# TzuYaoHuang/WaterLily.jl

Hardware: AMD Instinct MI355X
Metric: cells*steps/sec (3D TGV) ; smoother HBM GB/s vs peak (higher is better)
Workload: dtype f32; 1 GPU; 3D Taylor-Green vortex 512^3 Float32, wall-bounded, Re=1600, NoBody, remeasure=false (BASELINE configs[4] domain on 1 GPU); size=512, resjac=630, resjac_redo=0

## Files before the change

include/wlhip_bench.h:

```cpp
#ifndef WLHIP_BENCH_H
#define WLHIP_BENCH_H
#include "wlhip.h"
#ifdef __cplusplus
extern "C" {
#endif

enum { WL_PROF_GS_SWEEP = 0, WL_PROF_SMOOTH = 1, WL_PROF_JACOBI = 2, WL_PROF_CONVDIFF = 3, WL_PROF_RESIDUAL = 4,
       WL_PROF_BDIM = 5, WL_PROF_PROLONG = 6, WL_PROF_COARSE = 7, WL_PROF_STEP = 8, WL_PROF_GS_A = 9, WL_PROF_GS_B = 10, WL_PROF_NSLOTS = 11 };
int wl_prof_enable(int on);
int wl_prof_read(int slot, int* host_count, double* host_total_ms);

long wl_launch_count(void);
int wl_placement_scores(double* out, int cap);
int wl_sim_counter(wl_sim* s, const char* name, long* out);

#ifdef __cplusplus
}
#endif
#endif
```

waterlily.jl_amd/_lib.py:

```python
import ctypes as C
import os

_HERE = os.path.dirname(os.path.abspath(__file__))
LIB_PATH = os.environ.get("WLHIP_LIB") or os.path.join(_HERE, "libwlhip.so")


class wl_grid(C.Structure):
    _fields_ = [("D", C.c_int32), ("nx", C.c_int32), ("ny", C.c_int32), ("nz", C.c_int32),
                ("k0", C.c_int32), ("k1", C.c_int32), ("gk", C.c_int32), ("gnz", C.c_int32)]


class wl_body(C.Structure):
    _fields_ = [("kind", C.c_int32), ("c", C.c_float * 3), ("R", C.c_float), ("m", C.c_float * 3), ("V", C.c_float * 3)]


def make_body(body, D):
    name = body[0]
    pad = lambda v: [float(x) for x in v] + [0.0] * (3 - len(v))
    b = wl_body()
    if name == "sphere":
        b.kind, b.R, m, rest = 1, float(body[2]), [1.0] * D, body[3:]
    elif name == "cylinder":
        b.kind, b.R, m, rest = 1, float(body[2]), [0.0 if k == int(body[3]) else 1.0 for k in range(D)], body[4:]
    elif name == "plane":
# ... 138 lines not shown
    "wl_comm_set_periodic": (i32, [P, i32]),
    "wl_comm_halo_async": (i32, [P, P, G, i32, i32, P]),
    "wl_comm_combine_test": (i32, [P, P, P, P]),
    "wl_comm_destroy": (i32, [P]),
    "wl_comm_rank": (i32, [P]),
    "wl_comm_size": (i32, [P]),
    "wl_comm_stats": (i32, [P, C.POINTER(C.c_int64)]),
    "wl_halo_exchange": (i32, [P, P, G, i32, i32, P]),
    "wl_allgather_planes": (i32, [P, P, G, i32, P]),
    "wl_grid_slab": (i32, [G, i32, C.POINTER(C.c_int32), i32, i32, i32]),
    "wl_sim_create_slab": (i32, [C.POINTER(P), C.POINTER(wl_sim_desc), P]),
    "wl_launch_count": (C.c_long, []),
    "wl_reset_process_options": (i32, []),
    "wl_placement_scores": (i32, [C.POINTER(C.c_double), i32]),
    "wl_sim_counter": (i32, [P, C.c_char_p, C.POINTER(C.c_long)]),
    "wl_prof_enable": (i32, [i32]),
    "wl_prof_read": (i32, [i32, C.POINTER(i32), C.POINTER(f64)]),
    "wl_sim_pressure_force_sphere": (i32, [P, C.POINTER(f32), f32, C.POINTER(f64), P]),
    "wl_measure_body": (i32, [P, P, P, P, G, C.POINTER(wl_body), f32, i32, C.c_uint32, P]),
    "wl_pressure_force_body": (i32, [P, G, C.POINTER(wl_body), C.POINTER(f64), P]),
    "wl_viscous_force_body": (i32, [P, G, f32, C.POINTER(wl_body), C.POINTER(f64), P]),
    "wl_pressure_moment_body": (i32, [C.POINTER(f32), P, G, C.POINTER(wl_body), C.POINTER(f64), P]),
    "wl_viscous_moment_body": (i32, [C.POINTER(f32), P, G, f32, C.POINTER(wl_body), C.POINTER(f64), P]),
    "wl_sim_pressure_moment_body": (i32, [P, C.POINTER(f32), C.POINTER(wl_body), C.POINTER(f64), P]),
    "wl_sim_viscous_moment_body": (i32, [P, C.POINTER(f32), C.POINTER(wl_body), C.POINTER(f64), P]),
    "wl_sim_measure_body": (i32, [P, C.POINTER(wl_body), f32, P]),
    "wl_sim_pressure_force_body": (i32, [P, C.POINTER(wl_body), C.POINTER(f64), P]),
    "wl_sim_viscous_force_body": (i32, [P, C.POINTER(wl_body), C.POINTER(f64), P]),
    "wl_bodyset_measure_points": (i32, [C.POINTER(wl_bodyset), i32, C.POINTER(f32), i32, f32, C.POINTER(f32), C.POINTER(f32), C.POINTER(f32), P]),
    "wl_measure_bodyset": (i32, [P, P, P, P, G, C.POINTER(wl_bodyset), f32, i32, C.c_uint32, P]),
# ... 49 lines not shown
```

waterlily.jl_amd/csrc/wl_mg.hip:

```cpp
#include <cmath>
#include <cstdlib>
#include <utility>

#include "wl_common.hpp"
#include "wl_mg.hpp"

bool wl_mg_divisible(int n) { return (n % 2 == 0) && n > 4; }

int wl_mg::build(float* x, float* L, float* z, const wl_grid& g0, unsigned per, int maxlevels, wl_comm* c) {
  perdir = per; comm = (c && c->size > 1) ? c : nullptr;
  WL_TRY(wl_ctx_ensure());
  WL_HIP(hipMalloc(&red, wl_red_bytes()));
  ws = wl_red_ws(red);
  const bool dist0 = comm && g0.D == 3 && g0.nz != g0.gnz;
  if (dist0 && ((per >> 2) & 1u) && !comm->zperiodic) { wl_set_error("z-periodic z-slabs need a communicator in periodic mode (wl_comm_set_periodic)"); return WL_EINVAL; }
  std::vector<wl_grid> grids; std::vector<char> isdist; std::vector<wl_grid> views; std::vector<char> hasview;
  grids.push_back(g0); isdist.push_back(dist0); views.push_back(g0); hasview.push_back(0);
  while ((int)grids.size() <= maxlevels) {
    const wl_grid f = grids.back(); const bool fd = isdist.back();
    const bool cx = wl_mg_divisible(f.nx), cy = wl_mg_divisible(f.ny), cz = (f.D == 3) && wl_mg_divisible(f.gnz);
    if (!(cx || cy || cz)) break;
    wl_grid cgr = f; wl_grid vw = f; bool cd = fd, hv = false;
    if (cx) cgr.nx = 1 + f.nx / 2;
    if (cy) cgr.ny = 1 + f.ny / 2;
// ... 271 lines not shown
  }
  WL_TRY(halo(fine, fine.r, 1, s));
  if (l == 0 && shift_pending) { shift_pending = false; WL_TRY(wl::jacobi_pp_shift(fine.eps, fine.r, fine.x, fine.x_, 1.f, fine.cl, ws, WL_RD_L1_INIT, WL_RF_LINF_INIT, s)); }
  else {
    const int xz = fine.xzero ? 1 : 0; fine.xzero = false;
    if (zsplit_ranges(fine).on) {
      ZPart parts[3]; zsplit_parts(*this, fine, parts);
      for (int i = 0; i < 3; i++) if (parts[i].any()) WL_TRY(wl::jacobi_pp(fine.eps, fine.r, fine.x, fine.L, fine.D, fine.iD, parts[i].of(fine.x_), 1.f, *parts[i].cl, s, xz));
    } else WL_TRY(wl::jacobi_pp(fine.eps, fine.r, fine.x, fine.L, fine.D, fine.iD, fine.x_, 1.f, fine.cl, s, xz));
  }
  std::swap(fine.r, fine.eps);
  return 0;
}
int wl_mg::restrict_to_coarse(int l, bool to_tail, hipStream_t s) {
  Level& fine = lv[(size_t)l]; Level& coarse = lv[(size_t)l + 1];
  if (coarse.has_view) {
    WL_TRY(wl::restrict_(coarse.r, coarse.view, fine.r, fine.x_, s));
    WL_TRY(wl::allgather_planes(comm, coarse.r, coarse.view, 1, s));
  } else WL_TRY(wl::restrict_(coarse.r, coarse.x_, fine.r, fine.x_, s));
  coarse.xzero = skip_fill && !to_tail && l + 2 < (int)lv.size() && !perdir && !coarse.dist && !coarse.has_view;
  return coarse.xzero ? 0 : wl::fill(coarse.x, 0.f, (size_t)coarse.x_.cs, s);
}
int wl_mg::descend(int l, bool to_tail, float w, hipStream_t s) {
  Level& fine = lv[(size_t)l]; Level& coarse = lv[(size_t)l + 1];
  if (to_tail) WL_TRY(tail(l + 1, w, s));
  else {
    if (l + 2 < (int)lv.size()) WL_TRY(vcycle(l + 1, w, s, true));
    WL_TRY(smooth(l + 1, 4, w, s, false, nullptr, skip_r ? wl::B_XONLY : wl::B_BOTH));
  }
  return halo(coarse, coarse.x, 1, s, coarse_x_depth(fine, coarse));
}
// ... 96 lines not shown
```

waterlily.jl_amd/csrc/wl_mg.hpp:

```cpp
#pragma once
#include <algorithm>
#include <functional>
#include <vector>

#include "wl_comm.hpp"

bool wl_mg_divisible(int n);
struct WlNormSlots { int d, f; };
inline constexpr WlNormSlots WL_ZS_NORMS[3] = {{WL_RD_L1, WL_RF_LINF}, {WL_RD_L1_Z1, WL_RF_LINF_Z1}, {WL_RD_L1_Z2, WL_RF_LINF_Z2}};

struct wl_mg {
  struct Level {
    wl_grid g; GridX x_;
    float *L = nullptr, *D = nullptr, *iD = nullptr, *x = nullptr, *eps = nullptr, *r = nullptr, *z = nullptr;
    float *em = nullptr, *rs = nullptr;
    float* wx = nullptr;
    wl::ConstL cl{};
    bool xzero = false;
    bool part = false; int za = 0, zb = -1; wl::ConstL clp{};
    bool pend = false;
    bool dist = false;
    GridX view;
    bool has_view = false;
  };
// ... 18 lines not shown
  bool use_zsplit = true;
  long zsplit_min = 16L << 20;
  bool skip_fill = true;
  bool defer_shift = true;
  bool shift_pending = false;
  bool deep_halo = true;
  struct Spec {
    std::function<int(const float*)> tail; int check_head = 0; bool tail_stood = false, head_decided = false, head_due = false;
    void disarm() { tail = nullptr; check_head = 0; }
    void begin_solve(std::function<int(const float*)>* t, int* check) { t->swap(tail); *check = check_head; disarm(); tail_stood = head_decided = head_due = false; }
  } spec;
  int shift_path = -1;
  hipStream_t side = nullptr; hipEvent_t ev_decided = nullptr;
  double first_hd0 = 0.0;
  bool jacobi0_done = false;
  int norm_slots = 0;
  bool par_ranges = false;
  int x_halo_depth = 1;
  int last_xdefer = -1;
  bool use_xdefer = true;
  bool use_wide = true;
  bool overlap_smooth = true;
  bool use_tail = true;
  bool tail_ok(int first) const;
  int tail(int first, float w, hipStream_t s);
  float* slab = nullptr;
  void* red = nullptr;
  RedWs ws;
  std::vector<double> log_r1, log_rinf, log_w;

// ... 46 lines not shown
```

waterlily.jl_amd/csrc/wl_pdefer.hpp:

```cpp
#pragma once
#include "wl_common.hpp"

#ifdef __HIPCC__
__device__ __forceinline__ float wl_unscale(float x, float dt) { return x / dt; }
#endif

namespace wl {
int resjac(float* xout, float* rout, const float* x, const float* u, const GridX& g, float dt, float w, const ConstL& cl, const RedWs& ws, int slot_d, int slot_f, hipStream_t s,
           bool shell, const float* bcU, float dt_prev);
int project_unscale(float* u, const float* L, const float* x, float* pout, const GridX& g, float dt, const ConstL& cl, hipStream_t s, const BcFold* fold, bool skip_p);
int project_cfl(float* uout, const float* uin, const float* L, const float* x, float* pout, float* sigma, const GridX& g, float dt, const ConstL& cl, const RedWs& ws, int slot_f, hipStream_t s,
                int store_sigma, const BcFold* fold, bool skip_p);
}
```

waterlily.jl_amd/csrc/wl_resjac.hip:

```cpp
#include <cstdlib>

#include "wl_common.hpp"
#include "wl_pdefer.hpp"

namespace {

__device__ __forceinline__ float rj_cf(int Ia, int Na, float c) { return (Ia <= 2 || Ia >= Na) ? 0.f : c; }
__device__ __forceinline__ float rj_inv(float d) { return (d == 0.f) ? d : 1.0f / d; }
__device__ __forceinline__ float2 rj_ld2(const float* __restrict__ p, unsigned o) { return *reinterpret_cast<const float2*>(p + o); }
__device__ __forceinline__ void rj_st2(float* __restrict__ p, unsigned o, float2 v, bool s0, bool s1) {
  if (s0 && s1) *reinterpret_cast<float2*>(p + o) = v;
  else { if (s0) p[o] = v.x; if (s1) p[o + 1] = v.y; }
}
struct RjBc { int on; float U[3]; };
int g_resjac_on = 1;
long g_resjac_min = 6L << 20;

#define RJ_Y 32
#define RJ_NS rj32
#include "wl_resjac_body.inc"
#undef RJ_Y
#undef RJ_NS
#define RJ_Y 16
#define RJ_NS rj16
// ... 58 lines not shown
  return g_resjac_on && cl.on && g.D == 3 && (g.nz == g.gnz ? g.gk == 0 : (g.k0 >= 2 && g.nz - g.k1 >= 2 && g.k1 - g.k0 >= 8)) && (g.nx & 1) == 0 && g.nx >= 66 && g.ny >= 34 &&
         g.gnz >= 10 && g.cs < (1L << 30) && (long)(g.nx - 2) * (g.ny - 2) * (g.gnz - 2) >= g_resjac_min;
}
int shell_nonzero(const float* a, const GridX& g, int* dev_flag, hipStream_t s) {
  WL_HIP(hipMemsetAsync(dev_flag, 0, sizeof(int), s));
  hipLaunchKernelGGL(k_shell_nonzero, dim3(8, (unsigned)g.nz), dim3(WL_BLOCK), 0, s, g, a, dev_flag);
  int h = 1;
  WL_HIP(hipMemcpyAsync(&h, dev_flag, sizeof(int), hipMemcpyDeviceToHost, s));
  WL_HIP(hipStreamSynchronize(s));
  return h ? 1 : 0;
}
int resjac(float* xout, float* rout, const float* x, const float* u, const GridX& g, float dt, float w, const ConstL& cl, const RedWs& ws, int slot_d, int slot_f, hipStream_t s, bool shell, const float* bcU) {
  return resjac(xout, rout, x, u, g, dt, w, cl, ws, slot_d, slot_f, s, shell, bcU, 0.f);
}
int resjac(float* xout, float* rout, const float* x, const float* u, const GridX& g, float dt, float w, const ConstL& cl, const RedWs& ws, int slot_d, int slot_f, hipStream_t s, bool shell, const float* bcU, float dt_prev) {
  if (xout == x) { wl_set_error("resjac: output aliases input"); return WL_EINVAL; }
  const int np = g.k1 - g.k0;
  static const int rows_env = wl_exp_int("WL_RJ_ROWS", 0);
  const bool r16 = rows_env != 32;
  const int ntiles = r16 ? rj16::rj_tiles(g) : rj32::rj_tiles(g), per = (ntiles + 7) >> 3;
  const long SX = r16 ? rj16::rj_slots_per_xcd() : rj32::rj_slots_per_xcd();
  static const int envc = wl_exp_int("WL_RJ_CHUNK", 0);
  int zc = envc;
  if (zc <= 0) {
    static const int chforce = wl_exp_int("WL_RJ_CHUNKS", 0);
    double best = -1.0; zc = np;
    for (int chunks = 1; chunks <= np; chunks++) {
      const int z = (np + chunks - 1) / chunks;
      if (z < 8) break;
      const long W = (long)per * ((np + z - 1) / z), rounds = (W + SX - 1) / SX;
      double cost = (double)rounds * (z + 2) * (1.0 + 0.3 / (double)rounds);
      if (W < SX) cost = (z + 2) * 1.3;
      if (chforce > 0) cost = (chunks == chforce) ? 0.0 : 1e30;
      if (best < 0 || cost < best) { best = cost; zc = z; }
    }
  }
  if (zc > np) zc = np;
  const int nch = (np + zc - 1) / zc;
  const unsigned nb = (unsigned)(8 * per * nch);
  if (nb > WL_MAXPART) { wl_set_error("resjac: too many workgroups for the reduction workspace"); return WL_EINVAL; }
  if (dt_prev != 0.f && !(dt_prev > 0.f && dt > 0.f)) { wl_set_error("resjac: a pending unscale needs positive Δt"); return WL_EINVAL; }
  if (shell) hipLaunchKernelGGL(k_scale_shell, dim3(8, (unsigned)g.nz), dim3(WL_BLOCK), 0, s, g, xout, x, dt, dt_prev);
  RjBc bc{0, {0.f, 0.f, 0.f}};
  if (bcU) { if (g.nz != g.gnz) { wl_set_error("resjac: BC! on load is for the single domain"); return WL_EINVAL; } bc.on = 1; for (int a = 0; a < 3; a++) bc.U[a] = bcU[a]; }
  if (r16) rj16::rj_launch(nb, s, g, xout, rout, x, u, dt, dt_prev, w, cl, zc, ws.pa, ws.pb, ws.pm, bc);
  else rj32::rj_launch(nb, s, g, xout, rout, x, u, dt, dt_prev, w, cl, zc, ws.pa, ws.pb, ws.pm, bc);
  hipLaunchKernelGGL(k_resjac_fin, dim3(1), dim3(WL_BLOCK), 0, s, (const double*)ws.pa, (const double*)ws.pb, (const float*)ws.pm, (int)nb, ws.res_d, ws.res_f, slot_d, slot_f);
  WL_LAUNCH_CHECK(); return 0;
}
}
```

waterlily.jl_amd/csrc/wl_resjac_body.inc:

```
#define RJ_X 32
#define RJ_N (RJ_X * RJ_Y)
#define RJ_W (RJ_X + 2)
#define RJ_H ((RJ_Y + 2) * RJ_W)
#define RJ_SZ (2 * RJ_H)
#define RJ_HX 2
#define RJ_HY 2
#define RJ_CX (2 * RJ_X - 2 * RJ_HX)
#define RJ_CY (RJ_Y - 2 * RJ_HY)
namespace RJ_NS {
#ifndef RJ_WAVES
#define RJ_WAVES 8
#endif
template <int PEND>
__global__ void __launch_bounds__(RJ_N, RJ_WAVES) k_resjac(GridX g, float* __restrict__ xout, float* __restrict__ rout, const float* __restrict__ p, const float* __restrict__ u,
                                                    float dt, float dt_prev, float w, wl::ConstL cl, int zchunk, double* __restrict__ psum, double* __restrict__ pl1, float* __restrict__ pmax, RjBc bc) {
  __shared__ float sX[2][RJ_SZ];
  __shared__ float sE[2][RJ_SZ];
  const int ntx = (g.nx - 1 + RJ_CX - 1) / RJ_CX, nty = (g.ny - 2 + RJ_CY - 1) / RJ_CY;
  const int ntiles = ntx * nty;
  const unsigned h = blockIdx.x, q = h & 7u, sblk = h >> 3;
  const unsigned per = (unsigned)((ntiles + 7) >> 3);
  const int c = (int)(sblk / per);
  const int tl = (int)(q * per + (sblk - (unsigned)c * per));
  double nsum = 0.0, nl1 = 0.0; float nmax = 0.f;
  const int ks = g.k0 + c * zchunk, ke = (ks + zchunk < g.k1) ? ks + zchunk : g.k1;
  if (tl < ntiles && ks < ke) {
    const int tx = tl % ntx, ty = tl / ntx;
    const int lx = threadIdx.x % RJ_X, ly = threadIdx.x / RJ_X;
    const int i0 = tx * RJ_CX - RJ_HX + 2 * lx, j = 1 + ty * RJ_CY - RJ_HY + ly;
    const int lq = (ly + 1) * RJ_W + lx + 1;
    const bool indom = i0 >= 0 && i0 <= g.nx - 2 && j >= 0 && j < g.ny;
    const bool jin = j >= 1 && j <= g.ny - 2;
    const bool in0 = indom && jin && i0 >= 2, in1 = indom && jin && i0 + 1 <= g.nx - 2;
    const bool corep = 2 * lx >= RJ_HX && 2 * lx < 2 * RJ_X - RJ_HX && ly >= RJ_HY && ly < RJ_Y - RJ_HY;
    const bool st0 = corep && in0, st1 = corep && in1;
    const unsigned oc = indom ? (unsigned)i0 + (unsigned)j * (unsigned)g.sy : 0u;
    const unsigned sz = (unsigned)g.sz, cs = (unsigned)g.cs;
    for (int qq = threadIdx.x; qq < RJ_SZ; qq += RJ_N) { sX[0][qq] = 0.f; sX[1][qq] = 0.f; sE[0][qq] = 0.f; sE[1][qq] = 0.f; }
    const float cxa = rj_cf(i0 + 1, g.nx, cl.c[0]), cxb = rj_cf(i0 + 2, g.nx, cl.c[0]), cxc = rj_cf(i0 + 3, g.nx, cl.c[0]);
    const float ky = rj_cf(j + 1, g.ny, cl.c[1]), kyp = rj_cf(j + 2, g.ny, cl.c[1]);
    float dxy0 = 0.f; dxy0 -= (cxa + cxb); dxy0 -= (ky + kyp);
    float dxy1 = 0.f; dxy1 -= (cxb + cxc); dxy1 -= (ky + kyp);
    const float c2 = cl.c[2];
    const int oth0 = RJ_H + lq - 1, oth1 = lq + 1;
    auto plane_ok = [&](int K) { return K >= 0 && K <= g.nz - 1; };
    auto ldp = [&](int K) -> float2 {
      if (!(indom && plane_ok(K))) return make_float2(0.f, 0.f);
      const float2 v = rj_ld2(p, oc + (unsigned)K * sz);
      if (PEND) return make_float2(wl_unscale(v.x, dt_prev) * dt, wl_unscale(v.y, dt_prev) * dt);
      return make_float2(v.x * dt, v.y * dt);
    };
    const bool sbx = bc.on && (i0 == 0 || i0 == g.nx - 2);
    const bool sby = bc.on && j == 1, sbyp = bc.on && j + 1 == g.ny - 1;
    auto lduz = [&](int K) -> float2 {
      if (!(indom && plane_ok(K) && (in0 || in1))) return make_float2(0.f, 0.f);
      if (bc.on && (g.gk + K == 1 || g.gk + K == g.gnz - 1)) return make_float2(bc.U[2], bc.U[2]);
      return rj_ld2(u, 2u * cs + oc + (unsigned)K * sz);
    };
    const int K0 = ks - 1;
    float2 xm = ldp(K0 - 1), x0 = ldp(K0), xp;
    float2 uz0 = lduz(K0), uzp;
    float2 em1 = {0.f, 0.f}, e0 = em1, e1 = em1;
    float2 r1 = em1, r0 = em1;
    __syncthreads();
    sX[K0 & 1][lq] = x0.x; sX[K0 & 1][lq + RJ_H] = x0.y;
    for (int K = K0; K <= ke; K++) {
      xp = ldp(K + 1); uzp = lduz(K + 1);
      const bool planeK = g.gk + K >= 1 && g.gk + K <= g.gnz - 2 && K >= 1 && K <= g.nz - 2;
      float2 ux = {0.f, 0.f}, uy = ux, uyp = ux; float uxr = 0.f;
      if (planeK && (in0 || in1)) {
        const unsigned o = oc + (unsigned)K * sz;
        ux = rj_ld2(u, o); uxr = u[o + 2];
        uy = rj_ld2(u, cs + o); uyp = rj_ld2(u, cs + o + (unsigned)g.sy);
// ... 24 lines not shown
          e1.x = r0.x * id0;
        }
        if (in1) {
          float dv = 0.f;
          dv += uxr - ux.y;
          dv += uyp.y - uy.y;
          dv += uzp.y - uz0.y;
          float s = x0.y * d1;
          s += (x0.x * cxb + SX[oth1] * cxc);
          s += (SX[RJ_H + lq - RJ_W] * ky + SX[RJ_H + lq + RJ_W] * kyp);
          s += (xm.y * lz + xp.y * lzp);
          r0.y = (d1 == 0.f) ? 0.f : dv - s;
          e1.y = r0.y * id1;
        }
        if (K >= ks && K < ke) {
          const float a0 = st0 ? r0.x : 0.f, a1 = st1 ? r0.y : 0.f;
          nsum += (double)a0; nsum += (double)a1;
          nl1 += (double)fabsf(a0); nl1 += (double)fabsf(a1); nmax = fmaxf(nmax, fmaxf(fabsf(a0), fabsf(a1)));
        }
      }
      sE[K & 1][lq] = e1.x; sE[K & 1][lq + RJ_H] = e1.y;
      const int P = K - 1;
      if (P >= ks && P < ke && (st0 || st1)) {
        const float* __restrict__ SE = sE[P & 1];
        const float lzP = rj_cf(g.gk + P + 1, g.gnz, c2), lzpP = lz;
        const float zsP = lzP + lzpP;
        float2 rn, xn;
        {
          float s = e0.x * (dxy0 - zsP);
          s += (SE[oth0] * cxa + e0.y * cxb);
          s += (SE[lq - RJ_W] * ky + SE[lq + RJ_W] * kyp);
          s += (em1.x * lzP + e1.x * lzpP);
          rn.x = r1.x - w * s; xn.x = xm.x + w * e0.x;
        }
        {
          float s = e0.y * (dxy1 - zsP);
          s += (e0.x * cxb + SE[oth1] * cxc);
          s += (SE[RJ_H + lq - RJ_W] * ky + SE[RJ_H + lq + RJ_W] * kyp);
          s += (em1.y * lzP + e1.y * lzpP);
          rn.y = r1.y - w * s; xn.y = xm.y + w * e0.y;
        }
        const unsigned oP = oc + (unsigned)P * sz;
        rj_st2(rout, oP, rn, st0, st1);
        rj_st2(xout, oP, xn, st0, st1);
      }
      xm = x0; x0 = xp; uz0 = uzp;
    }
  }
  __shared__ double shs[RJ_N / 64], shl[RJ_N / 64]; __shared__ float shm[RJ_N / 64];
  nsum = wave_sum(nsum); nl1 = wave_sum(nl1); nmax = wave_max(nmax);
  __syncthreads();
  if ((threadIdx.x & 63) == 0) { shs[threadIdx.x >> 6] = nsum; shl[threadIdx.x >> 6] = nl1; shm[threadIdx.x >> 6] = nmax; }
  __syncthreads();
  if (threadIdx.x == 0) {
    double a = 0.0, l = 0.0; float mx = 0.f;
    for (int qq = 0; qq < RJ_N / 64; qq++) { a += shs[qq]; l += shl[qq]; mx = fmaxf(mx, shm[qq]); }
    psum[blockIdx.x] = a; pl1[blockIdx.x] = l; pmax[blockIdx.x] = mx;
  }
}
inline int rj_tiles(const GridX& g) { return ((g.nx - 1 + RJ_CX - 1) / RJ_CX) * ((g.ny - 2 + RJ_CY - 1) / RJ_CY); }
inline long rj_slots_per_xcd() { return 32L * (2048 / RJ_N); }
inline void rj_launch(unsigned nb, hipStream_t s, const GridX& g, float* xout, float* rout, const float* x, const float* u, float dt, float dt_prev, float w, const wl::ConstL& cl, int zc,
                      double* pa, double* pb, float* pm, const RjBc& bc) {
  if (dt_prev != 0.f) hipLaunchKernelGGL(k_resjac<1>, dim3(nb), dim3(RJ_N), 0, s, g, xout, rout, x, u, dt, dt_prev, w, cl, zc, pa, pb, pm, bc);
  else hipLaunchKernelGGL(k_resjac<0>, dim3(nb), dim3(RJ_N), 0, s, g, xout, rout, x, u, dt, dt_prev, w, cl, zc, pa, pb, pm, bc);
}
}
#undef RJ_X
#undef RJ_N
#undef RJ_W
#undef RJ_H
#undef RJ_SZ
#undef RJ_HX
#undef RJ_HY
#undef RJ_CX
#undef RJ_CY
```

waterlily.jl_amd/csrc/wl_sim.hip:

```cpp
#include <cmath>
#include <cstring>
#include <utility>
#include <vector>

#include "wl_common.hpp"
#include <algorithm>
#include "wl_mg.hpp"
#include "wl_body.hpp"
#include "wl_pdefer.hpp"
#include "wl_forces.hpp"
#include "wl_meanflow.hpp"
#include "wl_observe.hpp"

namespace {
template <int D>
__global__ void k_apply_tgv(GridX g, float* __restrict__ u, float kx, float ky, float kz) {
  int i, j; long m; int pz;
  wl_tile(g, m, pz);
  if (!cell_ij(g, m, i, j)) return;
  const int k = pz;
  const long o = m + (long)k * g.sz;
  const int I[3] = {i + 1, j + 1, (D == 3) ? g.gk + k + 1 : 1};
  for (int a = 0; a < D; a++) {
    float x[3];
// ... 274 lines not shown
        done->skips_p = wl::project_cfl_pair_path(G, l0.cl) && skip_p_now(c);
        WL_TRY(wl::project_cfl(us, u, mu0, p, ps, sigma, G, dtl, l0.cl, mg->ws, WL_RF_CFL, s, store_f ? 1 : 0, &fr, done->skips_p)); df.bc_folded = fr.on != 0;
        break;
      case Tail::SplitInPlace: WL_TRY(wl::project_unscale_split(u, mu0, p, ps, G, dtl, l0.cl, l0.clp, plan.z.na, plan.z.nb, s)); break;
      case Tail::Loader:
        done->skips_p = skip_p_now(c);
        if (!done->skips_p) WL_TRY(wl::div_scalar_to(ps, p, dtl, (size_t)G.cs, s));
        break;
      case Tail::InPlace:
        done->skips_p = skip_p_now(c);
        WL_TRY(wl::project_unscale(u, mu0, p, ps, G, dtl, l0.cl, s, &fr, done->skips_p)); df.bc_folded = fr.on != 0;
        break;
    }
    return 0;
  }
  struct Head { bool stood = false, solved = false, tail_ran = false, taken = false; double pre_r1 = 0.0; float pre_rinf = 0.f; };
  void head_swap() { swap_p(); std::swap(mg->lv[0].r, mg->lv[0].eps); }
  void head_take(Head* h) { head_swap(); mg->jacobi0_done = h->taken = true; }
  void head_accept(Head* h) {
    if (!h->taken) head_take(h);
    n_resjac++; resjac_redo_run = 0; h->stood = true; df.p_scale_pending = 0.f;
  }
  void head_discard(Head* h) {
    if (h->taken) { head_swap(); mg->jacobi0_done = h->taken = false; mg->n.pop_back(); }
    n_resjac_redo++;
    if (!resjac_force_redo && ++resjac_redo_run >= 3) resjac_backoff = true;
  }
  int head_speculate(const ProjCall& c, float dtl, const TailPlan& plan, TailDone* done, Head* h, hipStream_t s) {
    head_take(h);
    struct SpecClear { wl_mg* m; ~SpecClear() { m->spec.disarm(); } } spec_clear{mg};
    if (use_tailspec && plan.gateable) {
      mg->spec.tail = [&, dtl, done, s](const float* go) { return launch_tail(plan, c, dtl, go, done, s); };
      mg->spec.check_head = resjac_force_redo ? 2 : 1; n_tailspec_armed++;
    }
    const int slot = mg->rskip_slot, hist = slot >= 0 ? mg->rskip_hist[slot] : 0;
    WL_TRY(mg->solve(2e-3, itmx, nullptr, nullptr, nullptr, s, true, nullptr, nullptr));
    h->tail_ran = mg->spec.tail_stood; if (h->tail_ran) n_tailspec++;
    const bool due = mg->spec.head_decided ? mg->spec.head_due : (resjac_force_redo || wl_shift_due(mg->first_hd0, (double)wl_ninside_global(mg->lv[0].g)));
    if (due) { head_discard(h); if (slot >= 0) mg->rskip_hist[slot] = hist; }
    else { head_accept(h); h->solved = true; }
    return 0;
  }
  int head_read_back(Head* h, hipStream_t s) {
    WL_TRY(wl::combine_results(comm, mg->ws, s));
    double hd[WL_RD_COUNT]; float hf[WL_RF_COUNT]; WL_TRY(wl::read_results(mg->ws, hd, wl_upto(WL_RD_L1_INIT), hf, wl_upto(WL_RF_LINF_INIT), s));
    h->pre_r1 = hd[WL_RD_L1_INIT]; h->pre_rinf = hf[WL_RF_LINF_INIT];
    if (!wl_shift_due(hd[WL_RD_SUM], (double)wl_ninside_global(mg->lv[0].g)) && !resjac_force_redo) head_accept(h);
    else head_discard(h);
    return 0;
  }
  int head_fused(const ProjCall& c, float dtl, const TailPlan& plan, TailDone* done, Head* h, hipStream_t s) {
    { ProfScope pr(WL_PROF_RESIDUAL, s);
      if (comm) p_shell = 1;
      if (p_shell < 0) p_shell = (wl::shell_nonzero(p, G, (int*)(mg->ws.res_f + WL_RF_IFLAG), s) || wl::shell_nonzero(ps, G, (int*)(mg->ws.res_f + WL_RF_IFLAG), s)) ? 1 : 0;
      WL_TRY(wl::resjac(ps, mg->lv[0].eps, p, u, G, dtl, 1.f, mg->lv[0].cl, mg->ws, WL_RD_L1_INIT, WL_RF_LINF_INIT, s, p_shell != 0, df.bc_deferred ? d.uBC : nullptr, df.p_scale_pending)); }
    return use_headspec && !comm && itmx >= 1 ? head_speculate(c, dtl, plan, done, h, s) : head_read_back(h, s);
  }
  int head_two_kernel(float dtl, hipStream_t s) {
    wl_mg::Level& l0 = mg->lv[0];
    WL_TRY(settle(s));
    { ProfScope pr(WL_PROF_RESIDUAL, s);
      const ZSplit z = zsplit();
      if (z.on) WL_TRY(wl::div_residual_split(store_f ? sigma : nullptr, ps, l0.r, p, u, mu0, l0.D, l0.iD, G, dtl, mg->ws, l0.cl, l0.clp, z.na, z.nb, s));
      else WL_TRY(wl::div_residual(store_f ? sigma : nullptr, ps, l0.r, p, u, mu0, l0.D, l0.iD, G, dtl, mg->ws, l0.cl, s)); }
    swap_p();
    return 0;
  }
  int project_finish(const TailPlan& plan, const TailDone& done, float dtl, hipStream_t s) {
    df.bc_deferred = false;
    if (plan.form == Tail::Loader) { df.proj_pending = p; n_tailfuse++; }
    if (plan.form == Tail::PairCfl) {
      WL_TRY(wl::combine_results(comm, mg->ws, s));
      std::swap(u, us); df.cfl_done = true;
    }
    if (done.wide) n_tailwide++;
    if (done.skips_p) { df.p_scale_pending = dtl; n_pdefer++; }
    else swap_p();
    return plan.form == Tail::Loader ? 0 : bc_u(s);
  }
  int project_plain(float dtl, hipStream_t s) {
// ... 160 lines not shown
static double placement_score(wl_sim* s) {
  hipStream_t q = 0;
  const size_t n0 = s->mg->n.size();
  if (s->project(wl_sim::ProjCall::score(1.f, false), q) != 0) return 1e30;
  if (hipStreamSynchronize(q) != hipSuccess) return 1e30;
  hipEvent_t a, b; if (hipEventCreate(&a) != hipSuccess || hipEventCreate(&b) != hipSuccess) return 1e30;
  float ms = 1e30f; int rc = 0;
  for (int rep = 0; rep < 2 && rc == 0; rep++) {
    (void)hipEventRecord(a, q);
    rc = s->project(wl_sim::ProjCall::score(1.f, false), q); if (rc == 0) rc = s->project(wl_sim::ProjCall::score(0.5f, true), q);
    (void)hipEventRecord(b, q); (void)hipEventSynchronize(b);
    float t = 1e30f; (void)hipEventElapsedTime(&t, a, b);
    if (t < ms) ms = t;
  }
  (void)hipEventDestroy(a); (void)hipEventDestroy(b);
  s->mg->n.resize(n0); s->n_resjac = 0; s->n_resjac_redo = 0; s->resjac_redo_run = 0; s->resjac_backoff = false; s->df.cfl_done = false;
  s->mg->log_r1.clear(); s->mg->log_rinf.clear(); s->mg->log_w.clear();
  s->mg->rskip_hist[0] = s->mg->rskip_hist[1] = 0; s->mg->n_rskip = s->mg->n_rskip_redo = 0;
  return rc == 0 ? (double)ms : 1e30;
}
static double g_last_placement[8]; static int g_last_placement_n = 0;
int wl_sim_create(wl_sim** out, const wl_sim_desc* desc) {
  WL_CHECK(out && desc, "null pointer");
  static const int trials_env = [] { const char* e = getenv("WL_PLACEMENT_TRIALS"); const int v = e ? atoi(e) : 1; return v < 1 ? 1 : (v > 8 ? 8 : v); }();
  const bool owned = !desc->u && !desc->u0 && !desc->f && !desc->p && !desc->sigma && !desc->V && !desc->mu0 && !desc->mu1 && !desc->us;
  const long cells = (long)desc->dims[0] * desc->dims[1] * (desc->D == 3 ? desc->dims[2] : 1);
  int trials = (owned && desc->D == 3 && cells >= (48L << 20)) ? trials_env : 1;
  if (trials > 1) {
    size_t fr = 0, tot = 0;
    if (hipMemGetInfo(&fr, &tot) == hipSuccess) { const long fit = (long)(fr / 2 / ((size_t)cells * 160 + 1)); if (fit < trials) trials = fit < 1 ? 1 : (int)fit; }
  }
// ... 82 lines not shown
  if (n == "convt") { wl::conv_tile_enable(value != 0, value > 1 ? value : 0); return 0; }
  if (n == "pair") { wl::gsrb_pair_enable(value); return 0; }
  if (n == "fuse_p") { s->use_fuse_p = value != 0; return 0; }
  if (n == "zsplit_par") { s->mg->par_ranges = value != 0; return 0; }
  if (n == "itmx") { if (value < 1) { wl_set_error("itmx must be >= 1"); return WL_EINVAL; } s->itmx = value; return 0; }
  wl_set_error("unknown option " + n); return WL_EINVAL;
}
int wl_sim_update(wl_sim* s, void* st) { s->resjac_backoff = false; s->resjac_redo_run = 0; WL_TRY(s->refresh_body_mask(wl_stream(st))); return s->mg->update(wl_stream(st)); }

long wl_launch_count(void) { return g_wl_launches; }
int wl_reset_process_options(void) {
  wl::resjac_enable(1, 6L << 20); wl::conv_tile_min(2048); wl::conv_tile_enable(1, 0); wl::conv_flux_enable(1); wl::tail_lds_enable(1); wl::conv_body_tile_enable(1);
  wl::gsrb_pair_enable(1); wl::jacobi_march_enable(1); wl::conv_march_enable(0);
  return 0;
}
int wl_sim_counter(wl_sim* s, const char* name, long* out) {
  WL_CHECK(s && name && out, "bad argument");
  const std::string n(name);
  if (n == "resjac") { *out = s->n_resjac; return 0; }
  if (n == "resjac_redo") { *out = s->n_resjac_redo; return 0; }
  if (n == "resjac_backoff") { *out = s->resjac_backoff ? 1 : 0; return 0; }
  if (n == "tailfuse") { *out = s->n_tailfuse; return 0; }
  if (n == "tailfuse_min") { *out = s->tailfuse_min; return 0; }
  if (n == "bcdefer") { *out = s->n_bcdefer; return 0; }
  if (n == "pdefer") { *out = s->n_pdefer; return 0; }
  if (n == "tailwide") { *out = s->n_tailwide; return 0; }
  if (n == "rskip") { *out = s->mg->n_rskip; return 0; }
  if (n == "rskip_redo") { *out = s->mg->n_rskip_redo; return 0; }
  if (n == "tailspec") { *out = s->n_tailspec; return 0; }
  if (n == "tailspec_armed") { *out = s->n_tailspec_armed; return 0; }
  if (n == "xdefer") { *out = s->mg->last_xdefer; return 0; }
  if (n == "abwide") { *out = s->mg->n_wide; return 0; }
  if (n == "hybrid") { *out = s->n_hybrid; return 0; }
  if (n == "body_tile") { *out = wl::conv_body_tile_launches(); return 0; }
  if (n == "mask_valid") { *out = s->mask_valid ? 1 : 0; return 0; }
  if (n == "mask_near") { *out = s->census.near; return 0; }
  if (n == "mask_needf_only") { *out = s->census.needf_only; return 0; }
  if (n == "mask_m0var_only") { *out = s->census.m0var_only; return 0; }
  if (n == "mask_clean_in_box") { *out = s->census.clean_in_box; return 0; }
  if (n == "dirty_z0") { *out = s->dirty_z[0]; return 0; }
  if (n == "dirty_z1") { *out = s->dirty_z[1]; return 0; }
// ... 230 lines not shown
```

waterlily.jl_amd/simulation.py:

```python
import ctypes as C

import numpy as np

from . import core
from ._lib import WlError, check, lib, wl_grid, wl_sim_desc
from .core import perdir_mask, ptr, stream
from .flow import Flow, mom_step_
from .poisson import MultiLevelPoisson


def _is_set(body):
    from .bodies import AbstractBody
    return isinstance(body, AbstractBody)


def _x0(x0, D):
    return None if x0 is None else (C.c_float * 3)(*([float(v) for v in x0] + [0.0] * (3 - D)))


def _as_set(body):
    from .bodies import Body
    if _is_set(body):
        return body
    if isinstance(body, (tuple, list)) and body and isinstance(body[0], str):
# ... 292 lines not shown
                else:
                    check(lib().wl_sim_update(self._h, stream()))
            self.mom_step_()
            return
        n = 0
        while self.sim_time() < t_end and n < max_steps:
            self.sim_step_(remeasure=remeasure)
            n += 1

    def update_(self):
        check(lib().wl_sim_update(self._h, stream()))

    def set_option(self, name, value):
        check(lib().wl_sim_set_option(self._h, name.encode(), int(value)))

    def counter(self, name):
        v = C.c_long(0)
        check(lib().wl_sim_counter(self._h, name.encode(), C.byref(v)))
        return int(v.value)

    @property
    def dt(self):
        out = (C.c_float * 1000000)()
        k = lib().wl_sim_dt(self._h, out, 1000000)
        return [np.float32(v) for v in out[:k]]

    def time(self):
        return lib().wl_sim_time(self._h)

    def sim_time(self):
# ... 269 lines not shown
```

Before: 17.45 billion cells*steps/s.

## Fuse level-0 residual restriction into the resjac head kernel

The fused residual/Jacobi head kernel now stages each tile's new residual in shared memory and sums 2x2x2 blocks into the coarse-level residual. Partial sums are carried across z-plane pairs in shared memory. Tiles shrink in x so every fine cell is owned by exactly one tile, and the z chunk size is rounded to even. The multigrid V-cycle then skips its separate level-0 restrict kernel, saving a full re-read of the fine residual. This costs extra shared memory, narrower tiles, and extra in-kernel work, and it is on by default only for grids of at least 128M interior cells, single-domain and non-periodic.

```diff
diff --git a/include/wlhip_bench.h b/include/wlhip_bench.h
--- a/include/wlhip_bench.h
+++ b/include/wlhip_bench.h
@@ -13,6 +13,8 @@
 long wl_launch_count(void);
 int wl_placement_scores(double* out, int cap);
 int wl_sim_counter(wl_sim* s, const char* name, long* out);
+int wl_sim_set_headrst(wl_sim* s, int on);
+int wl_sim_head_restrict(wl_sim* s, float dt, float dt_prev, float* r_out, float* rc_out, void* stream);
 
 #ifdef __cplusplus
 }
diff --git a/waterlily.jl_amd/_lib.py b/waterlily.jl_amd/_lib.py
--- a/waterlily.jl_amd/_lib.py
+++ b/waterlily.jl_amd/_lib.py
@@ -176,6 +176,8 @@
     "wl_reset_process_options": (i32, []),
     "wl_placement_scores": (i32, [C.POINTER(C.c_double), i32]),
     "wl_sim_counter": (i32, [P, C.c_char_p, C.POINTER(C.c_long)]),
+    "wl_sim_set_headrst": (i32, [P, i32]),
+    "wl_sim_head_restrict": (i32, [P, f32, f32, P, P, P]),
     "wl_prof_enable": (i32, [i32]),
     "wl_prof_read": (i32, [i32, C.POINTER(i32), C.POINTER(f64)]),
     "wl_sim_pressure_force_sphere": (i32, [P, C.POINTER(f32), f32, C.POINTER(f64), P]),
diff --git a/waterlily.jl_amd/csrc/wl_mg.hip b/waterlily.jl_amd/csrc/wl_mg.hip
--- a/waterlily.jl_amd/csrc/wl_mg.hip
+++ b/waterlily.jl_amd/csrc/wl_mg.hip
@@ -309,7 +309,10 @@
 }
 int wl_mg::restrict_to_coarse(int l, bool to_tail, hipStream_t s) {
   Level& fine = lv[(size_t)l]; Level& coarse = lv[(size_t)l + 1];
-  if (coarse.has_view) {
+  const bool done = l == 0 && restrict0_done;
+  if (l == 0) restrict0_done = false;
+  if (done) { if (coarse.has_view) { wl_set_error("restrict_to_coarse: the head's restrict! is for a single-domain level"); return WL_EINVAL; } }
+  else if (coarse.has_view) {
     WL_TRY(wl::restrict_(coarse.r, coarse.view, fine.r, fine.x_, s));
     WL_TRY(wl::allgather_planes(comm, coarse.r, coarse.view, 1, s));
   } else WL_TRY(wl::restrict_(coarse.r, coarse.x_, fine.r, fine.x_, s));
diff --git a/waterlily.jl_amd/csrc/wl_mg.hpp b/waterlily.jl_amd/csrc/wl_mg.hpp
--- a/waterlily.jl_amd/csrc/wl_mg.hpp
+++ b/waterlily.jl_amd/csrc/wl_mg.hpp
@@ -56,6 +56,7 @@
   hipStream_t side = nullptr; hipEvent_t ev_decided = nullptr;
   double first_hd0 = 0.0;
   bool jacobi0_done = false;
+  bool restrict0_done = false;
   int norm_slots = 0;
   bool par_ranges = false;
   int x_halo_depth = 1;
diff --git a/waterlily.jl_amd/csrc/wl_pdefer.hpp b/waterlily.jl_amd/csrc/wl_pdefer.hpp
--- a/waterlily.jl_amd/csrc/wl_pdefer.hpp
+++ b/waterlily.jl_amd/csrc/wl_pdefer.hpp
@@ -8,6 +8,10 @@
 namespace wl {
 int resjac(float* xout, float* rout, const float* x, const float* u, const GridX& g, float dt, float w, const ConstL& cl, const RedWs& ws, int slot_d, int slot_f, hipStream_t s,
            bool shell, const float* bcU, float dt_prev);
+struct HeadRst { float* rc; GridX gc; int ran; };
+bool resjac_rst_ok(const GridX& g, const GridX& gc);
+int resjac(float* xout, float* rout, const float* x, const float* u, const GridX& g, float dt, float w, const ConstL& cl, const RedWs& ws, int slot_d, int slot_f, hipStream_t s,
+           bool shell, const float* bcU, float dt_prev, HeadRst* rst);
 int project_unscale(float* u, const float* L, const float* x, float* pout, const GridX& g, float dt, const ConstL& cl, hipStream_t s, const BcFold* fold, bool skip_p);
 int project_cfl(float* uout, const float* uin, const float* L, const float* x, float* pout, float* sigma, const GridX& g, float dt, const ConstL& cl, const RedWs& ws, int slot_f, hipStream_t s,
                 int store_sigma, const BcFold* fold, bool skip_p);
diff --git a/waterlily.jl_amd/csrc/wl_resjac.hip b/waterlily.jl_amd/csrc/wl_resjac.hip
--- a/waterlily.jl_amd/csrc/wl_resjac.hip
+++ b/waterlily.jl_amd/csrc/wl_resjac.hip
@@ -96,20 +96,32 @@
   return resjac(xout, rout, x, u, g, dt, w, cl, ws, slot_d, slot_f, s, shell, bcU, 0.f);
 }
 int resjac(float* xout, float* rout, const float* x, const float* u, const GridX& g, float dt, float w, const ConstL& cl, const RedWs& ws, int slot_d, int slot_f, hipStream_t s, bool shell, const float* bcU, float dt_prev) {
+  return resjac(xout, rout, x, u, g, dt, w, cl, ws, slot_d, slot_f, s, shell, bcU, dt_prev, nullptr);
+}
+bool resjac_rst_ok(const GridX& g, const GridX& gc) {
+  return g.D == 3 && g.nz == g.gnz && g.gk == 0 && g.k0 == 1 && g.k1 == g.nz - 1 && gc.D == 3 && gc.nz == gc.gnz && gc.gk == 0 && gc.k0 == 1 && gc.k1 == gc.nz - 1 &&
+         ((g.nx | g.ny | g.nz) & 1) == 0 && gc.nx - 2 == (g.nx - 2) / 2 && gc.ny - 2 == (g.ny - 2) / 2 && gc.nz - 2 == (g.nz - 2) / 2 && gc.cs < (1L << 31);
+}
+int resjac(float* xout, float* rout, const float* x, const float* u, const GridX& g, float dt, float w, const ConstL& cl, const RedWs& ws, int slot_d, int slot_f, hipStream_t s, bool shell, const float* bcU, float dt_prev,
+           HeadRst* rst) {
   if (xout == x) { wl_set_error("resjac: output aliases input"); return WL_EINVAL; }
   const int np = g.k1 - g.k0;
+  bool rs = rst && rst->rc && resjac_rst_ok(g, rst->gc);
+  if (rst) rst->ran = 0;
   static const int rows_env = wl_exp_int("WL_RJ_ROWS", 0);
   const bool r16 = rows_env != 32;
-  const int ntiles = r16 ? rj16::rj_tiles(g) : rj32::rj_tiles(g), per = (ntiles + 7) >> 3;
+  static const int envc = wl_exp_int("WL_RJ_CHUNK", 0);
+  if (envc > 0 && (envc & 1) && envc < np) rs = false;
+  const int ntiles = r16 ? rj16::rj_tiles(g, rs) : rj32::rj_tiles(g, rs), per = (ntiles + 7) >> 3;
   const long SX = r16 ? rj16::rj_slots_per_xcd() : rj32::rj_slots_per_xcd();
-  static const int envc = wl_exp_int("WL_RJ_CHUNK", 0);
   int zc = envc;
   if (zc <= 0) {
     static const int chforce = wl_exp_int("WL_RJ_CHUNKS", 0);
     double best = -1.0; zc = np;
     for (int chunks = 1; chunks <= np; chunks++) {
-      const int z = (np + chunks - 1) / chunks;
+      int z = (np + chunks - 1) / chunks;
       if (z < 8) break;
+      if (rs) z += z & 1;
       const long W = (long)per * ((np + z - 1) / z), rounds = (W + SX - 1) / SX;
       double cost = (double)rounds * (z + 2) * (1.0 + 0.3 / (double)rounds);
       if (W < SX) cost = (z + 2) * 1.3;
@@ -125,8 +137,10 @@
   if (shell) hipLaunchKernelGGL(k_scale_shell, dim3(8, (unsigned)g.nz), dim3(WL_BLOCK), 0, s, g, xout, x, dt, dt_prev);
   RjBc bc{0, {0.f, 0.f, 0.f}};
   if (bcU) { if (g.nz != g.gnz) { wl_set_error("resjac: BC! on load is for the single domain"); return WL_EINVAL; } bc.on = 1; for (int a = 0; a < 3; a++) bc.U[a] = bcU[a]; }
-  if (r16) rj16::rj_launch(nb, s, g, xout, rout, x, u, dt, dt_prev, w, cl, zc, ws.pa, ws.pb, ws.pm, bc);
-  else rj32::rj_launch(nb, s, g, xout, rout, x, u, dt, dt_prev, w, cl, zc, ws.pa, ws.pb, ws.pm, bc);
+  float* rc = rs ? rst->rc : nullptr;
+  if (r16) rj16::rj_launch(nb, s, g, xout, rout, x, u, dt, dt_prev, w, cl, zc, ws.pa, ws.pb, ws.pm, bc, rc);
+  else rj32::rj_launch(nb, s, g, xout, rout, x, u, dt, dt_prev, w, cl, zc, ws.pa, ws.pb, ws.pm, bc, rc);
+  if (rs) rst->ran = 1;
   hipLaunchKernelGGL(k_resjac_fin, dim3(1), dim3(WL_BLOCK), 0, s, (const double*)ws.pa, (const double*)ws.pb, (const float*)ws.pm, (int)nb, ws.res_d, ws.res_f, slot_d, slot_f);
   WL_LAUNCH_CHECK(); return 0;
 }
diff --git a/waterlily.jl_amd/csrc/wl_resjac_body.inc b/waterlily.jl_amd/csrc/wl_resjac_body.inc
--- a/waterlily.jl_amd/csrc/wl_resjac_body.inc
+++ b/waterlily.jl_amd/csrc/wl_resjac_body.inc
@@ -7,16 +7,25 @@
 #define RJ_HY 2
 #define RJ_CX (2 * RJ_X - 2 * RJ_HX)
 #define RJ_CY (RJ_Y - 2 * RJ_HY)
+#define RJ_RX (RJ_CX - 2)
+#define RJ_NC ((RJ_RX / 2) * (RJ_CY / 2))
 namespace RJ_NS {
 #ifndef RJ_WAVES
 #define RJ_WAVES 8
 #endif
-template <int PEND>
+#ifndef RJ_RST_PARTS
+#define RJ_RST_PARTS 3
+#endif
+template <int PEND, int RST>
 __global__ void __launch_bounds__(RJ_N, RJ_WAVES) k_resjac(GridX g, float* __restrict__ xout, float* __restrict__ rout, const float* __restrict__ p, const float* __restrict__ u,
-                                                    float dt, float dt_prev, float w, wl::ConstL cl, int zchunk, double* __restrict__ psum, double* __restrict__ pl1, float* __restrict__ pmax, RjBc bc) {
+                                                    float dt, float dt_prev, float w, wl::ConstL cl, int zchunk, double* __restrict__ psum, double* __restrict__ pl1, float* __restrict__ pmax, RjBc bc, float* __restrict__ rc) {
+  constexpr int CX = RST ? RJ_RX : RJ_CX;
+  constexpr bool RSTAGE = RST != 0 && (RJ_RST_PARTS & 1) != 0, RSUM = RST != 0 && (RJ_RST_PARTS & 2) != 0;
+  __shared__ __align__(8) float sR[RST ? 2 : 1][RST ? RJ_CY * RJ_RX : 2];
+  __shared__ float sC[RST ? RJ_NC : 1];
   __shared__ float sX[2][RJ_SZ];
   __shared__ float sE[2][RJ_SZ];
-  const int ntx = (g.nx - 1 + RJ_CX - 1) / RJ_CX, nty = (g.ny - 2 + RJ_CY - 1) / RJ_CY;
+  const int ntx = (g.nx - 1 + CX - 1) / CX, nty = (g.ny - 2 + RJ_CY - 1) / RJ_CY;
   const int ntiles = ntx * nty;
   const unsigned h = blockIdx.x, q = h & 7u, sblk = h >> 3;
   const unsigned per = (unsigned)((ntiles + 7) >> 3);
@@ -27,13 +36,14 @@
   if (tl < ntiles && ks < ke) {
     const int tx = tl % ntx, ty = tl / ntx;
     const int lx = threadIdx.x % RJ_X, ly = threadIdx.x / RJ_X;
-    const int i0 = tx * RJ_CX - RJ_HX + 2 * lx, j = 1 + ty * RJ_CY - RJ_HY + ly;
+    const int i0 = tx * CX - RJ_HX + 2 * lx, j = 1 + ty * RJ_CY - RJ_HY + ly;
     const int lq = (ly + 1) * RJ_W + lx + 1;
     const bool indom = i0 >= 0 && i0 <= g.nx - 2 && j >= 0 && j < g.ny;
     const bool jin = j >= 1 && j <= g.ny - 2;
     const bool in0 = indom && jin && i0 >= 2, in1 = indom && jin && i0 + 1 <= g.nx - 2;
     const bool corep = 2 * lx >= RJ_HX && 2 * lx < 2 * RJ_X - RJ_HX && ly >= RJ_HY && ly < RJ_Y - RJ_HY;
     const bool st0 = corep && in0, st1 = corep && in1;
+    const bool own0 = st0 && (!RST || lx >= 2), own1 = st1 && (!RST || lx <= RJ_X - 3);
     const unsigned oc = indom ? (unsigned)i0 + (unsigned)j * (unsigned)g.sy : 0u;
     const unsigned sz = (unsigned)g.sz, cs = (unsigned)g.cs;
     for (int qq = threadIdx.x; qq < RJ_SZ; qq += RJ_N) { sX[0][qq] = 0.f; sX[1][qq] = 0.f; sE[0][qq] = 0.f; sE[1][qq] = 0.f; }
@@ -57,6 +67,29 @@
       if (bc.on && (g.gk + K == 1 || g.gk + K == g.gnz - 1)) return make_float2(bc.U[2], bc.U[2]);
       return rj_ld2(u, 2u * cs + oc + (unsigned)K * sz);
     };
+    auto rj_restrict = [&](int Q) {
+      const bool lo = ly < RJ_HY, hi = ly >= RJ_Y - RJ_HY;
+      if ((lo || hi) && lx < RJ_RX / 2) {
+        int t = threadIdx.x; asm volatile("" : "+v"(t));
+        const int lx = t % RJ_X, ly = t / RJ_X;
+        const int hr = lo ? ly : ly - (RJ_Y - 2 * RJ_HY);
+        const int I = tx * (RJ_RX / 2) + 1 + lx;
+        const int cnx = (g.nx >> 1) + 1, cny = (g.ny >> 1) + 1;
+#pragma unroll 1
+        for (int m = 0; m < (RJ_CY / 2 + 2 * RJ_HY - 1) / (2 * RJ_HY); m++) {
+          const int cj = hr + 2 * RJ_HY * m, J = ty * (RJ_CY / 2) + 1 + cj;
+          if (cj < RJ_CY / 2 && I <= cnx - 2 && J <= cny - 2) {
+            const float* __restrict__ SR = sR[Q & 1] + 2 * cj * RJ_RX + 2 * lx;
+            const float2 a = *reinterpret_cast<const float2*>(SR), b = *reinterpret_cast<const float2*>(SR + RJ_RX);
+            float s = 0.f;
+            if (!(Q & 1)) s = sC[cj * (RJ_RX / 2) + lx];
+            s += a.x; s += a.y; s += b.x; s += b.y;
+            if (Q & 1) sC[cj * (RJ_RX / 2) + lx] = s;
+            else rc[(unsigned)I + ((unsigned)J + (unsigned)(Q >> 1) * (unsigned)cny) * (unsigned)cnx] = s;
+          }
+        }
+      }
+    };
     const int K0 = ks - 1;
     float2 xm = ldp(K0 - 1), x0 = ldp(K0), xp;
     float2 uz0 = lduz(K0), uzp;
@@ -111,7 +144,7 @@
           e1.y = r0.y * id1;
         }
         if (K >= ks && K < ke) {
-          const float a0 = st0 ? r0.x : 0.f, a1 = st1 ? r0.y : 0.f;
+          const float a0 = own0 ? r0.x : 0.f, a1 = own1 ? r0.y : 0.f;
           nsum += (double)a0; nsum += (double)a1;
           nl1 += (double)fabsf(a0); nl1 += (double)fabsf(a1); nmax = fmaxf(nmax, fmaxf(fabsf(a0), fabsf(a1)));
         }
@@ -140,9 +173,16 @@
         const unsigned oP = oc + (unsigned)P * sz;
         rj_st2(rout, oP, rn, st0, st1);
         rj_st2(xout, oP, xn, st0, st1);
+        if (RSTAGE) {
+          float* __restrict__ SR = sR[P & 1] + (ly - RJ_HY) * RJ_RX + 2 * lx - 3;
+          if (own0) SR[0] = rn.x;
+          if (own1) SR[1] = rn.y;
+        }
       }
       xm = x0; x0 = xp; uz0 = uzp;
+      if (RSUM && K - 2 >= ks) rj_restrict(K - 2);
     }
+    if (RSUM) { __syncthreads(); rj_restrict(ke - 1); }
   }
   __shared__ double shs[RJ_N / 64], shl[RJ_N / 64]; __shared__ float shm[RJ_N / 64];
   nsum = wave_sum(nsum); nl1 = wave_sum(nl1); nmax = wave_max(nmax);
@@ -155,12 +195,15 @@
     psum[blockIdx.x] = a; pl1[blockIdx.x] = l; pmax[blockIdx.x] = mx;
   }
 }
-inline int rj_tiles(const GridX& g) { return ((g.nx - 1 + RJ_CX - 1) / RJ_CX) * ((g.ny - 2 + RJ_CY - 1) / RJ_CY); }
+inline int rj_tiles(const GridX& g, bool rst) { const int cx = rst ? RJ_RX : RJ_CX; return ((g.nx - 1 + cx - 1) / cx) * ((g.ny - 2 + RJ_CY - 1) / RJ_CY); }
 inline long rj_slots_per_xcd() { return 32L * (2048 / RJ_N); }
 inline void rj_launch(unsigned nb, hipStream_t s, const GridX& g, float* xout, float* rout, const float* x, const float* u, float dt, float dt_prev, float w, const wl::ConstL& cl, int zc,
-                      double* pa, double* pb, float* pm, const RjBc& bc) {
-  if (dt_prev != 0.f) hipLaunchKernelGGL(k_resjac<1>, dim3(nb), dim3(RJ_N), 0, s, g, xout, rout, x, u, dt, dt_prev, w, cl, zc, pa, pb, pm, bc);
-  else hipLaunchKernelGGL(k_resjac<0>, dim3(nb), dim3(RJ_N), 0, s, g, xout, rout, x, u, dt, dt_prev, w, cl, zc, pa, pb, pm, bc);
+                      double* pa, double* pb, float* pm, const RjBc& bc, float* rc) {
+  if (rc) {
+    if (dt_prev != 0.f) hipLaunchKernelGGL((k_resjac<1, 1>), dim3(nb), dim3(RJ_N), 0, s, g, xout, rout, x, u, dt, dt_prev, w, cl, zc, pa, pb, pm, bc, rc);
+    else hipLaunchKernelGGL((k_resjac<0, 1>), dim3(nb), dim3(RJ_N), 0, s, g, xout, rout, x, u, dt, dt_prev, w, cl, zc, pa, pb, pm, bc, rc);
+  } else if (dt_prev != 0.f) hipLaunchKernelGGL((k_resjac<1, 0>), dim3(nb), dim3(RJ_N), 0, s, g, xout, rout, x, u, dt, dt_prev, w, cl, zc, pa, pb, pm, bc, rc);
+  else hipLaunchKernelGGL((k_resjac<0, 0>), dim3(nb), dim3(RJ_N), 0, s, g, xout, rout, x, u, dt, dt_prev, w, cl, zc, pa, pb, pm, bc, rc);
 }
 }
 #undef RJ_X
@@ -172,3 +215,5 @@
 #undef RJ_HY
 #undef RJ_CX
 #undef RJ_CY
+#undef RJ_RX
+#undef RJ_NC
diff --git a/waterlily.jl_amd/csrc/wl_sim.hip b/waterlily.jl_amd/csrc/wl_sim.hip
--- a/waterlily.jl_amd/csrc/wl_sim.hip
+++ b/waterlily.jl_amd/csrc/wl_sim.hip
@@ -312,17 +312,28 @@
     }
     return 0;
   }
-  struct Head { bool stood = false, solved = false, tail_ran = false, taken = false; double pre_r1 = 0.0; float pre_rinf = 0.f; };
+  struct Head { bool stood = false, solved = false, tail_ran = false, taken = false, rst = false; double pre_r1 = 0.0; float pre_rinf = 0.f; };
   void head_swap() { swap_p(); std::swap(mg->lv[0].r, mg->lv[0].eps); }
-  void head_take(Head* h) { head_swap(); mg->jacobi0_done = h->taken = true; }
+  void head_take(Head* h) { head_swap(); mg->jacobi0_done = h->taken = true; mg->restrict0_done = h->rst; }
   void head_accept(Head* h) {
     if (!h->taken) head_take(h);
     n_resjac++; resjac_redo_run = 0; h->stood = true; df.p_scale_pending = 0.f;
+    if (h->rst) n_headrst++;
   }
   void head_discard(Head* h) {
-    if (h->taken) { head_swap(); mg->jacobi0_done = h->taken = false; mg->n.pop_back(); }
+    if (h->taken) { head_swap(); mg->jacobi0_done = mg->restrict0_done = h->taken = false; mg->n.pop_back(); }
     n_resjac_redo++;
     if (!resjac_force_redo && ++resjac_redo_run >= 3) resjac_backoff = true;
+  }
+  int use_headrst = -1;
+  long headrst_min = 128L << 20;
+  long n_headrst = 0;
+  bool headrst_ok() const {
+    const wl_mg::Level& c = mg->lv[1];
+    static const int env = wl_exp_int("WL_HEADRST", -1);
+    const int mode = use_headrst >= 0 ? use_headrst : env;
+    const bool on = mode < 0 ? (long)(G.nx - 2) * (G.ny - 2) * (G.gnz - 2) >= headrst_min : mode != 0;
+    return on &&!comm && !d.perdir_mask && !mg->perdir && itmx >= 1 && !c.dist && !c.has_view && wl::resjac_rst_ok(G, c.x_);
   }
   int head_speculate(const ProjCall& c, float dtl, const TailPlan& plan, TailDone* done, Head* h, hipStream_t s) {
     head_take(h);
@@ -351,7 +362,9 @@
     { ProfScope pr(WL_PROF_RESIDUAL, s);
       if (comm) p_shell = 1;
       if (p_shell < 0) p_shell = (wl::shell_nonzero(p, G, (int*)(mg->ws.res_f + WL_RF_IFLAG), s) || wl::shell_nonzero(ps, G, (int*)(mg->ws.res_f + WL_RF_IFLAG), s)) ? 1 : 0;
-      WL_TRY(wl::resjac(ps, mg->lv[0].eps, p, u, G, dtl, 1.f, mg->lv[0].cl, mg->ws, WL_RD_L1_INIT, WL_RF_LINF_INIT, s, p_shell != 0, df.bc_deferred ? d.uBC : nullptr, df.p_scale_pending)); }
+      wl::HeadRst rst{headrst_ok() ? mg->lv[1].r : nullptr, mg->lv[1].x_, 0};
+      WL_TRY(wl::resjac(ps, mg->lv[0].eps, p, u, G, dtl, 1.f, mg->lv[0].cl, mg->ws, WL_RD_L1_INIT, WL_RF_LINF_INIT, s, p_shell != 0, df.bc_deferred ? d.uBC : nullptr, df.p_scale_pending, &rst));
+      h->rst = rst.ran != 0; }
     return use_headspec && !comm && itmx >= 1 ? head_speculate(c, dtl, plan, done, h, s) : head_read_back(h, s);
   }
   int head_two_kernel(float dtl, hipStream_t s) {
@@ -362,6 +375,17 @@
       if (z.on) WL_TRY(wl::div_residual_split(store_f ? sigma : nullptr, ps, l0.r, p, u, mu0, l0.D, l0.iD, G, dtl, mg->ws, l0.cl, l0.clp, z.na, z.nb, s));
       else WL_TRY(wl::div_residual(store_f ? sigma : nullptr, ps, l0.r, p, u, mu0, l0.D, l0.iD, G, dtl, mg->ws, l0.cl, s)); }
     swap_p();
+    return 0;
+  }
+  int head_restrict_probe(float dtl, float dt_prev, float* r_out, float* rc_out, hipStream_t s) {
+    WL_TRY(settle(s));
+    if (df.proj_pending || !head_fused_path() || !headrst_ok()) { wl_set_error("wl_sim_head_restrict: the restricting head does not run on this handle"); return WL_EINVAL; }
+    wl_mg::Level& l0 = mg->lv[0]; wl_mg::Level& l1 = mg->lv[1];
+    wl::HeadRst rst{l1.r, l1.x_, 0};
+    WL_TRY(wl::resjac(ps, l0.eps, p, u, G, dtl, 1.f, l0.cl, mg->ws, WL_RD_L1_INIT, WL_RF_LINF_INIT, s, true, nullptr, dt_prev, &rst));
+    if (!rst.ran) { wl_set_error("wl_sim_head_restrict: the launcher declined"); return WL_EINVAL; }
+    WL_HIP(hipMemcpyAsync(r_out, l0.eps, sizeof(float) * (size_t)G.cs, hipMemcpyDeviceToDevice, s));
+    WL_HIP(hipMemcpyAsync(rc_out, l1.r, sizeof(float) * (size_t)l1.x_.cs, hipMemcpyDeviceToDevice, s));
     return 0;
   }
   int project_finish(const TailPlan& plan, const TailDone& done, float dtl, hipStream_t s) {
@@ -552,7 +576,7 @@
     if (t < ms) ms = t;
   }
   (void)hipEventDestroy(a); (void)hipEventDestroy(b);
-  s->mg->n.resize(n0); s->n_resjac = 0; s->n_resjac_redo = 0; s->resjac_redo_run = 0; s->resjac_backoff = false; s->df.cfl_done = false;
+  s->mg->n.resize(n0); s->n_resjac = 0; s->n_resjac_redo = 0; s->n_headrst = 0; s->resjac_redo_run = 0; s->resjac_backoff = false; s->df.cfl_done = false;
   s->mg->log_r1.clear(); s->mg->log_rinf.clear(); s->mg->log_w.clear();
   s->mg->rskip_hist[0] = s->mg->rskip_hist[1] = 0; s->mg->n_rskip = s->mg->n_rskip_redo = 0;
   return rc == 0 ? (double)ms : 1e30;
@@ -665,6 +689,11 @@
   wl::gsrb_pair_enable(1); wl::jacobi_march_enable(1); wl::conv_march_enable(0);
   return 0;
 }
+int wl_sim_set_headrst(wl_sim* s, int on) { WL_CHECK(s, "bad argument"); s->use_headrst = on < 0 ? -1 : (on != 0 ? 1 : 0); return 0; }
+int wl_sim_head_restrict(wl_sim* s, float dt, float dt_prev, float* r_out, float* rc_out, void* st) {
+  WL_CHECK(s && r_out && rc_out && dt > 0.f && dt_prev >= 0.f, "bad argument");
+  return s->head_restrict_probe(dt, dt_prev, r_out, rc_out, wl_stream(st));
+}
 int wl_sim_counter(wl_sim* s, const char* name, long* out) {
   WL_CHECK(s && name && out, "bad argument");
   const std::string n(name);
@@ -676,6 +705,7 @@
   if (n == "bcdefer") { *out = s->n_bcdefer; return 0; }
   if (n == "pdefer") { *out = s->n_pdefer; return 0; }
   if (n == "tailwide") { *out = s->n_tailwide; return 0; }
+  if (n == "headrst") { *out = s->n_headrst; return 0; }
   if (n == "rskip") { *out = s->mg->n_rskip; return 0; }
   if (n == "rskip_redo") { *out = s->mg->n_rskip_redo; return 0; }
   if (n == "tailspec") { *out = s->n_tailspec; return 0; }
diff --git a/waterlily.jl_amd/simulation.py b/waterlily.jl_amd/simulation.py
--- a/waterlily.jl_amd/simulation.py
+++ b/waterlily.jl_amd/simulation.py
@@ -330,6 +330,15 @@
     def set_option(self, name, value):
         check(lib().wl_sim_set_option(self._h, name.encode(), int(value)))
 
+    def set_headrst(self, on):
+        check(lib().wl_sim_set_headrst(self._h, int(on)))
+
+    def head_restrict(self, dt, dt_prev=0.0):
+        r = core.jl_zeros(self.Ng)
+        rc = core.jl_zeros(tuple((n - 2) // 2 + 2 for n in self.Ng))
+        check(lib().wl_sim_head_restrict(self._h, float(dt), float(dt_prev), ptr(r), ptr(rc), stream()))
+        return r, rc
+
     def counter(self, name):
         v = C.c_long(0)
         check(lib().wl_sim_counter(self._h, name.encode(), C.byref(v)))
```

Result: no change. 17.53 billion cells*steps/s (median of 6 runs) (+0.4%).
